# soedinglab/spacedust

Measured on AMD Instinct MI355X. Metric: clustersearch throughput (genome-pairs/s; SW GCUPS alongside), higher is better.
Workload: dtype int16

## Files before the change

### include/spacedust_gpu.h

```cpp
#ifndef SPACEDUST_GPU_H
#define SPACEDUST_GPU_H

#include <stddef.h>
#include <stdint.h>

#ifdef __cplusplus
extern "C" {
#endif

enum {
    SD_OK = 0,
    SD_ENODEVICE = -1,
    SD_EHIP = -2,
    SD_EINVAL = -3,
    SD_ENOMEM = -4,
    SD_EUNSUPPORTED = -5,
    SD_EMISMATCH = -6
};

typedef struct sd_ctx sd_ctx;
typedef struct sd_seqset sd_seqset;
typedef struct sd_target sd_target;

int sd_ctx_create(int device, sd_ctx **out);
// ... 59 lines not shown
                                    uint32_t nPairs, const uint32_t *pairQ, const uint32_t *pairT, const uint16_t *pairDiag,
                                    const uint8_t *isIdentity, float seqIdThr, int32_t alnLenThr, uint32_t *outIdx, sd_sw_result *out,
                                    uint32_t *nOut, char *btPool, uint64_t btCap, uint64_t *btUsed);

int sd_sw_align_alt_batch(sd_ctx *ctx, const sd_sw_params *par, const sd_seqset *queries, const sd_seqset *targets, uint32_t nSeeds,
                          const uint32_t *seedQ, const uint32_t *seedT, const int32_t *tStart, const int32_t *tEnd,
                          const uint8_t *isIdentity, uint32_t maxAlt, float seqIdThr, int32_t alnLenThr, int32_t seqIdMode,
                          sd_sw_result *out, uint32_t *outCount, char *btPool, uint64_t btCap, uint64_t *btUsed);
int sd_sw_alt_last_stats(sd_ctx *ctx, uint64_t *groups, uint64_t *seedRounds, uint64_t *bytesCopied);

int sd_sw_set_cigar_pool(sd_ctx *ctx, int on);
int sd_sw_download_bytes(sd_ctx *ctx, uint64_t *recordBytes, uint64_t *poolBytes);

int sd_sw_set_narrow_final(sd_ctx *ctx, int on);
int sd_sw_set_shared_start(sd_ctx *ctx, int on);

int sd_selftest_sort_pairs(sd_ctx *ctx, const uint32_t *keys, const uint32_t *vals, uint32_t n, int beginBit, int endBit, uint32_t *outKeys,
                           uint32_t *outVals);
int sd_selftest_scan(sd_ctx *ctx, const uint32_t *in, uint32_t n, uint64_t *exclusiveSum, uint32_t *runningMax);
int sd_selftest_score_class(int kernel , int32_t n, int32_t tL, int shared, int32_t wideRowLimit,
                            uint32_t *klass, char *scope, size_t cap);
int sd_selftest_r2p_weights(sd_ctx *ctx, uint32_t nTasks, const uint32_t *nRows, const uint32_t *L, const uint8_t *cells, float *freq,
                            float *eff);

int sd_sw_align_batch_hostpath(sd_ctx *ctx, const sd_sw_params *par, const sd_seqset *queries, const sd_seqset *targets,
                               uint32_t nPairs, const uint32_t *pairQ, const uint32_t *pairT, const uint8_t *isIdentity,
                               sd_sw_result *out, char *btPool, uint64_t btCap, uint64_t *btUsed);

int sd_sw_score_batch(sd_ctx *ctx, const sd_sw_params *par, const sd_seqset *queries, const sd_seqset *targets,
                      uint32_t nPairs, const uint32_t *pairQ, const uint32_t *pairT, int lanes, int reverse,
                      const int32_t *qEnd, const int32_t *tEnd, int32_t *out);

int sd_sw_last_cells(sd_ctx *ctx, uint64_t *forwardCells, uint64_t *reverseCells, uint64_t *tracebackCells);

typedef struct {
    int32_t kmerSize;
// ... 419 lines not shown
```

### spacedust_amd/_lib.py

```python
import ctypes as C
import os

import numpy as np

HERE = os.path.dirname(os.path.abspath(__file__))
LIB_PATH = os.path.join(HERE, 'libsdgpu.so')

_vp = C.c_void_p


SD_OK, SD_ENODEVICE, SD_EHIP, SD_EINVAL, SD_ENOMEM, SD_EUNSUPPORTED, SD_EMISMATCH = 0, -1, -2, -3, -4, -5, -6


class SdError(RuntimeError):
    pass


class SwParams(C.Structure):
    _fields_ = [('gapOpen', C.c_int32), ('gapExtend', C.c_int32), ('matrix', C.c_int8 * 441), ('covMode', C.c_int32),
                ('covThr', C.c_float), ('evalThr', C.c_double), ('swMode', C.c_int32), ('dbResidues', C.c_uint64)]


class SwResult(C.Structure):
    _fields_ = [('score', C.c_int32), ('qStart', C.c_int32), ('qEnd', C.c_int32), ('tStart', C.c_int32),
# ... 223 lines not shown
        'sd_search_result_arrays': (C.c_int, [_vp] + [_vp] * 12),
        'sd_search_result_write_tsv': (C.c_int, [_vp, C.c_char_p, C.c_char_p, _vp, C.c_char_p, _vp, C.c_char_p, _vp, C.c_char_p, _vp,
                                                 C.c_int, C.c_int, C.c_uint64, C.POINTER(C.c_uint64), C.POINTER(C.c_uint64)]),
        'sd_search_result_records': (C.c_int, [_vp, _vp, C.c_uint64, C.POINTER(C.c_uint64)]),
        'sd_agg_records': (C.c_int, [_vp] * 7 + [_vp, C.c_uint64, C.POINTER(C.c_uint64)]),
        'sd_records_check': (C.c_int, [_vp, C.c_uint64, C.c_uint32, C.c_uint32, C.c_uint32, C.c_uint32, C.POINTER(C.c_uint64), C.POINTER(C.c_uint64)]),
        'sd_records_write_tsv': (C.c_int, [_vp, C.c_uint64, C.c_char_p, C.c_int, C.c_uint64, C.c_char_p, _vp, C.c_char_p, _vp, C.c_char_p, _vp,
                                           C.c_char_p, _vp, C.c_int, C.POINTER(C.c_uint64), C.POINTER(C.c_uint64)]),
        'sd_search_result_destroy': (None, [_vp]),
        'sd_search_stats': (C.c_int, [_vp, _vp, _vp]),
        'sd_search_download_bytes': (C.c_int, [_vp, C.POINTER(C.c_uint64), C.POINTER(C.c_uint64)]),
        'sd_sw_set_cigar_pool': (C.c_int, [_vp, C.c_int]),
        'sd_sw_download_bytes': (C.c_int, [_vp, C.POINTER(C.c_uint64), C.POINTER(C.c_uint64)]),
        'sd_sw_set_narrow_final': (C.c_int, [_vp, C.c_int]),
        'sd_sw_set_shared_start': (C.c_int, [_vp, C.c_int]),
        'sd_r2p_create': (C.c_int, [C.POINTER(_vp)]),
        'sd_r2p_destroy': (None, [_vp]),
        'sd_r2p_batch': (C.c_int, [_vp, C.POINTER(R2pParams), C.c_uint32] + [_vp] * 12),
        'sd_r2p_batch_device': (C.c_int, [_vp, _vp, C.POINTER(R2pParams), C.c_uint32] + [_vp] * 12),
        'sd_selftest_r2p_weights': (C.c_int, [_vp, C.c_uint32, _vp, _vp, _vp, _vp, _vp]),
        'sd_selftest_score_class': (C.c_int, [C.c_int, C.c_int32, C.c_int32, C.c_int, C.c_int32, C.POINTER(C.c_uint32), C.c_char_p, C.c_size_t]),
        'sd_shard_query_sets': (C.c_int, [_vp, C.c_uint32, C.c_uint32, C.c_uint32, _vp, C.POINTER(C.c_uint32)]),
        'sd_comm_unique_id': (C.c_int, [C.c_char_p]),
        'sd_comm_init': (C.c_int, [C.c_int, C.c_int, C.c_int, C.c_char_p, C.POINTER(_vp)]),
        'sd_comm_destroy': (None, [_vp]),
        'sd_comm_host_buffer': (C.c_int, [_vp, C.c_int, C.c_uint64, C.POINTER(_vp)]),
        'sd_comm_last_error': (C.c_char_p, [_vp]),
        'sd_search_set_records_sink': (C.c_int, [_vp, _vp, _vp]),
        'sd_gather_stream_begin': (C.c_int, [_vp, C.c_int, C.c_uint32, _vp, C.c_uint32, _vp, C.c_uint64, C.c_int, C.POINTER(_vp)]),
        'sd_gather_stream_end': (C.c_int, [_vp, _vp, _vp, C.POINTER(C.c_uint64)]),
# ... 61 lines not shown
```

### spacedust_amd/api.py

```python
import ctypes as C

import numpy as np

from . import _lib
from .cpus import effective_cpus
from ._lib import SdError, ptr


def _check(ctx, rc, what):
    if rc != 0:
        msg = ''
        if ctx is not None:
            msg = _lib.load().sd_last_error(ctx).decode(errors='replace')
        raise SdError('%s failed (%d): %s' % (what, rc, msg))


class Host:

    def __init__(self, threads=0):
        import os
        self.L = _lib.load()
        self.threads = threads or effective_cpus()
        h = C.c_void_p()
        _check(None, self.L.sd_host_create(self.threads, C.byref(h)), 'sd_host_create')
# ... 81 lines not shown
        return out

    def evalue(self, db_residues, score, qlen):
        return self.L.sd_host_evalue(db_residues, float(score), float(qlen))

    def bitscore(self, score):
        return self.L.sd_host_bitscore(float(score))

    def score_class(self, kernel, n, tl, shared, wide_row_limit):
        klass = C.c_uint32()
        if not hasattr(self, '_scope_buf'):
            self._scope_buf = C.create_string_buffer(48)
        _check(None, self.L.sd_selftest_score_class(kernel, n, tl, int(shared), wide_row_limit, C.byref(klass), self._scope_buf, 48),
               'sd_selftest_score_class')
        return klass.value, self._scope_buf.value.decode()


def uncompress_cigar(c):
    out, n = [], 0
    for ch in c:
        if '0' <= ch <= '9':
            n = n * 10 + ord(ch) - 48
        else:
            out.append(ch * (n if n else 1))
            n = 0
    return ''.join(out)


def swapresults(entries, first_db_residues, second_db_keys, eval_thr=0.001, gap_open=11, gap_extend=1, want_counts=False):
    L = _lib.load()
# ... 333 lines not shown
        out = np.zeros(len(hq), _lib.RESCORE_DTYPE)
        _check(self.h, self.L.sd_rescore_diagonal_batch(self.h, C.byref(par), queries.h, targets.h, len(hq), ptr(hq), ptr(ht), ptr(hd),
                                                        ptr(out)), 'sd_rescore_diagonal_batch')
        return out

    def set_cigar_pool(self, on=True):
        _check(self.h, self.L.sd_sw_set_cigar_pool(self.h, 1 if on else 0), 'sd_sw_set_cigar_pool')
        self._cigar_pool = bool(on)

    def set_narrow_final(self, on=True):
        _check(self.h, self.L.sd_sw_set_narrow_final(self.h, 1 if on else 0), 'sd_sw_set_narrow_final')

    def set_shared_start(self, on=True):
        _check(self.h, self.L.sd_sw_set_shared_start(self.h, 1 if on else 0), 'sd_sw_set_shared_start')

    def sw_download_bytes(self):
        a, b = C.c_uint64(), C.c_uint64()
        self.L.sd_sw_download_bytes(self.h, C.byref(a), C.byref(b))
        return a.value, b.value

    def sw_cells(self):
        f, r, t = C.c_uint64(), C.c_uint64(), C.c_uint64()
        self.L.sd_sw_last_cells(self.h, C.byref(f), C.byref(r), C.byref(t))
        return f.value, r.value, t.value

    def __del__(self):
        try:
            h, self.h = self.h, None
            if h:
                self.L.sd_ctx_destroy(h)
# ... 483 lines not shown
```

### spacedust_amd/csrc/cli/sd_mod_iter.cpp

```cpp
#include "sd_align_core.h"
#include "sd_cli.h"
#include "sd_pref_core.h"

#include <algorithm>
#include <atomic>
#include <chrono>
#include <climits>
#include <cmath>
#include <condition_variable>
#include <cstdio>
#include <cstdlib>
#include <cstring>
#include <memory>
#include <mutex>
#include <omp.h>
#include <string>
#include <sys/resource.h>
#include <thread>
#include <vector>

namespace sdcli {

namespace {

// ... 43 lines not shown

struct Worker {
    sd_ctx *ctx = nullptr;
    sd_host *host = nullptr;
    sd_r2p *r2p = nullptr;
    int threads = 1;
    QueryChunk Q;
    std::vector<uint8_t> failed;
    AlignChunk C;
    std::vector<uint32_t> mark;
    uint32_t stamp = 0;
    ~Worker() {
        if (r2p) sd_r2p_destroy(r2p);
        if (ctx) sd_sw_set_narrow_final(ctx, 0);
        if (ctx) sd_sw_set_shared_start(ctx, 0);
        if (ctx) sd_ctx_destroy(ctx);
        if (host) sd_host_destroy(host);
    }
};

double quantE(double v) {
    char text[32];
    double back = v;
    sd_host_quantise_3e(v, text, &back);
    return back;
}

int failChunk(ChunkOut &o, int rc, const std::string &what, sd_ctx *ctx) {
    o.rc = rc;
    o.err = what + " failed (" + std::to_string(rc) + ")";
// ... 255 lines not shown
    nWorkers = std::max(1, std::min(nWorkers, 8));
    uint32_t chunkQ = (uint32_t) std::max<long long>(1, a.integer("--iter-chunk-queries", getenv("SD_ITER_CHUNK") ? atoi(getenv("SD_ITER_CHUNK")) : 1500));
    const int perWorker = std::max(1, std::min(threads, (threads * 3 / 2 + nWorkers - 1) / nWorkers));
    std::vector<std::unique_ptr<Worker> > workers;
    for (int w = 0; w < nWorkers; w++) {
        workers.emplace_back(new Worker());
        Worker &W = *workers.back();
        W.threads = perWorker;
        int rc = sd_ctx_create(device, &W.ctx);
        if (rc != SD_OK) return failNoDevice(rc);
        if (sd_host_create(perWorker, &W.host) != SD_OK) return fail("sd_host_create failed");
        if (sd_r2p_create(&W.r2p) != SD_OK) return fail("sd_r2p_create failed");
        if (S.profile) sd_profile_enable(W.ctx, 1);
        sd_sw_set_narrow_final(W.ctx, (getenv("SD_SW_NARROW_FINAL") && atoi(getenv("SD_SW_NARROW_FINAL")) == 0) ? 0 : 1);
        sd_sw_set_shared_start(W.ctx, (getenv("SD_SW_SHARED_START") && atoi(getenv("SD_SW_SHARED_START")) == 0) ? 0 : 1);
    }
    uint64_t indexEntries = 0;
    TargetH seqTarget, profTarget;
    SeqSetH tset;
    {
        sd_ctx *c0 = workers[0]->ctx;
        uint64_t st[2] = {0, 0};
        if (int rc = buildTarget(host.h, c0, S.pfSeq, tdb->residues.data(), tdb->offsets.data(), tdb->n, &seqTarget.t, st)) return rc;
        indexEntries = st[0];
        info(a, "Index table k-mer threshold: %d at k-mer size %d\nIndex statistics\nEntries:          %llu\n", S.pfSeq.kmerThr, S.pfSeq.k,
             (unsigned long long) st[0]);
        if (numIt > 1) {
            if (int rc = buildTarget(host.h, c0, S.pfProf, tdb->residues.data(), tdb->offsets.data(), tdb->n, &profTarget.t, st, std::string(),
                                     "sd_target_build (profile searches)"))
                return rc;
// ... 420 lines not shown
```

### spacedust_amd/csrc/hip/sd_common.h

```cpp
#ifndef SD_COMMON_H
#define SD_COMMON_H

#include <hip/hip_runtime.h>

#include <cstdarg>
#include <cstdint>
#include <cstdio>
#include <cstring>
#include <algorithm>
#include <ctime>
#include <sys/prctl.h>
#include <map>
#include <mutex>
#include <string>
#include <vector>

#include "spacedust_gpu.h"

struct sd_profile_entry {
    double ms = 0.0;
    uint64_t launches = 0;
};

struct sd_ctx {
    int device = 0;
    hipStream_t stream = nullptr;
    std::string lastError;
    bool profiling = false;
    std::map<std::string, sd_profile_entry> profile;
    hipEvent_t evStart = nullptr, evStop = nullptr;
    bool biasTablesUploaded = false;
    hipEvent_t evSync = nullptr;
    uint64_t cellsFwd = 0, cellsRev = 0, cellsTb = 0;
    uint64_t cellsUngapped = 0;
    uint64_t altGroups = 0, altSeedRounds = 0, altBytes = 0;
    const sd_sw_result *alignDevRes = nullptr;
    size_t alignDevResN = 0;
    bool cigarPool = false;
    bool sharedStart = false;
    bool narrowFinal = false;
    uint64_t d2hRecordBytes = 0, d2hPoolBytes = 0;
    struct ExpandState {
        uint64_t nPairs = 0, runsRead = 0, bytesWritten = 0;
        uint32_t nAB = 0;
        const int32_t *abStartA = nullptr, *abStartB = nullptr, *bcStartB = nullptr, *bcStartC = nullptr;
        const uint64_t *abRunOff = nullptr, *bcRowOff = nullptr, *bcRunOff = nullptr, *pairOff = nullptr;
        const uint32_t *abRuns = nullptr, *bcRuns = nullptr, *abCluster = nullptr;
        const sd_expand_result *res = nullptr;
    } expand;
    hipDeviceProp_t prop;
    struct WsEntry { void *p = nullptr; size_t bytes = 0; };
    std::map<std::string, WsEntry> ws;
    std::map<std::string, WsEntry> pinned;
    struct ProfPending { std::string name; hipEvent_t a = nullptr, b = nullptr; };
// ... 343 lines not shown
```

### spacedust_amd/csrc/hip/sd_sw.hip

```cpp
#include "sd_common.h"
#include <unistd.h>


#include <algorithm>
#include <cmath>
#include <cstring>
#include <memory>
#include <omp.h>
#include <numeric>

#include "../host/sd_host.h"
#include "sd_sw_pk.h"

namespace {

using sdpk::SwTask;
using sdpk::NARROW_EXACT;

template <int RT>
__global__ void __launch_bounds__(64)
sw_score_kernel(const SwTask *__restrict__ tasks, uint32_t nTasks, const uint8_t *__restrict__ qRes,
                const int8_t *__restrict__ qBias, const uint8_t *__restrict__ tRes, const int8_t *__restrict__ mat,
                int go, int ge, int32_t *__restrict__ out, uint2 *__restrict__ boundary,
                const uint32_t *__restrict__ order ,
// ... 451 lines not shown
        }
        going = going && !bad && (i > 0 || j > 0);
    }
    if (!have || l != 0) return;
    if (bad || i != 0 || j != 0) {
        res[2 * id] = -1;
        return;
    }
    ids += (q[0] == t[0]);
    *--o = 'M';
    len++;
    res[2 * id] = len;
    res[2 * id + 1] = ids;
}

template <bool PROF>
__global__ void __launch_bounds__(64)
sw_traceback_narrow_kernel(TbTask *__restrict__ tasks, uint32_t nTasks, const uint8_t *__restrict__ qRes,
                           const int8_t *__restrict__ qBias, const uint8_t *__restrict__ tRes, const int8_t *__restrict__ mat,
                           int go, int ge, int qCap, int tCap, char *__restrict__ bt, int32_t *__restrict__ res,
                           const uint32_t *__restrict__ order, const int8_t *__restrict__ qProf ) {
    extern __shared__ uint8_t ldsRaw[];
    __shared__ int8_t smat[441];
    for (int i = threadIdx.x; i < 441; i += 64) smat[i] = mat[i];
    const int grp = threadIdx.x >> 5, l = threadIdx.x & 31;
    const uint32_t lid = blockIdx.x * 2 + grp;
    const bool have = lid < nTasks;
    const uint32_t id = have ? (order ? order[lid] : lid) : 0;
    TbTask tk;
    if (have) tk = tasks[id];
    else { tk.qLen = 0; tk.tLen = 0; tk.band = 1; tk.score = 0; tk.maxv = 0; tk.qAbs = 0; tk.tAbs = 0; tk.slot = 0; tk.dirOff = 0; tk.btOff = 0; }
    const int qLen = tk.qLen, tLen = tk.tLen;
    const size_t perTask = (size_t) 16 * qCap + 2 * (size_t) qCap + tCap;
    uint8_t *dirs = ldsRaw + grp * perTask;
    uint8_t *sq = dirs + (size_t) 16 * qCap;
    int8_t *scb = (int8_t *) (sq + qCap);
    uint8_t *st = (uint8_t *) (scb + qCap);
    for (int x = l; x < qLen; x += 32) {
        sq[x] = qRes[tk.qAbs + x];
        scb[x] = qBias[tk.qAbs + x];
    }
    for (int x = l; x < tLen; x += 32) st[x] = tRes[tk.tAbs + x];
    __syncthreads();

    const int NEG = -(1 << 28);
    int band = tk.band, maxv = tk.maxv;
    bool reached = false;
    for (;;) {
        const int width = band * 2 + 3;
        const bool fits = width <= 32;
        int hb = 0, eb = 0;
        const int rows = (fits && !reached) ? qLen : 0;
        const int rowsOther = __shfl_xor(rows, 32, 64);
        const int nRows = max(rows, rowsOther);
        auto cellOps = [&](int row, int &qv, int &tv, int &cbv) {
            int r = row < qLen ? row : qLen - 1;
            r = r > 0 ? r : 0;
            const int x0 = (r - band) > 0 ? (r - band) : 0;
            int jn = x0 + l - 1;
            jn = jn >= tLen ? tLen - 1 : jn;
            jn = jn > 0 ? jn : 0;
            tv = st[jn];
            qv = 0;
            cbv = 0;
            if (!PROF) {
                qv = sq[r];
                cbv = scb[r];
            }
        };
        auto cellLook = [&](int row, int qv, int tv) -> int {
            int r = row < qLen ? row : qLen - 1;
            r = r > 0 ? r : 0;
            if (PROF) return (int) qProf[(tk.qAbs + (uint64_t) r) * 21 + (tv < 21 ? tv : 20)];
            return (int) smat[21 * qv + tv];
        };
        int qb, tb, cbb;
        cellOps(0, qb, tb, cbb);
        int sNext = cellLook(0, qb, tb), cNext = cbb;
        cellOps(1, qb, tb, cbb);
        for (int i = 0; i < nRows; i++) {
            const bool live = i < rows;
            const int sCur = sNext, cCur = cNext;
            sNext = cellLook(i + 1, qb, tb);
            cNext = cbb;
            cellOps(i + 2, qb, tb, cbb);
            const int xi = (i - band) > 0 ? (i - band) : 0;
            const int delta = (i - band) >= 1 ? 1 : 0;
            int end = tLen - 1;
            end = end < i + band ? end : i + band;
            const int edge = end + 1 < width - 1 ? end + 1 : width - 1;
            const int W = end - xi + 1;
            const bool zeroed = live && (l == 0 || l == edge);
            hb = zeroed ? 0 : hb;
            eb = zeroed ? 0 : eb;
            const int hbUp = dppZ(hb, 0x130), ebUp = dppZ(eb, 0x130), hbDn = dppZ(hb, 0x138);
            const int hE = delta ? hbUp : hb, eE = delta ? ebUp : eb, hD = delta ? hb : hbDn;
            const int u = l;
            const bool valid = live && u >= 1 && u <= W;
            const int t1 = i == 0 ? -go : hE - go;
            const int t2 = i == 0 ? -ge : eE - ge;
            const int eNew = t1 > t2 ? t1 : t2;
            const bool dirE = t1 > t2;
            const int e1 = eNew > 0 ? eNew : 0;
            const int diag = hD + sCur + cCur;
            const int T = e1 > diag ? e1 : diag;
            int incl = valid ? T + ge * u + 1 : 0, o;
            o = dppZ(incl, 0x111); incl = incl > o ? incl : o;
            o = dppZ(incl, 0x112); incl = incl > o ? incl : o;
            o = dppZ(incl, 0x114); incl = incl > o ? incl : o;
            o = dppZ(incl, 0x118); incl = incl > o ? incl : o;
            o = dppI(0, incl, 0x142, 0xa); incl = incl > o ? incl : o;
            int excl = dppZ(incl, 0x138);
            excl = l == 0 ? 0 : excl;
            const int gx = excl - go - 1;
            const int g = (-ge) > gx ? (-ge) : gx;
            const int f = g - ge * (u - 1);
            const int hcv = T > f ? T : f;
            int hcP = dppZ(hcv, 0x138), fP = dppZ(f, 0x138);
            hcP = u <= 1 ? 0 : hcP;
            fP = u <= 1 ? 0 : fP;
            const bool dirF = (hcP - go) > (fP - ge);
            const int f1 = f > 0 ? f : 0;
            const int tmp1 = e1 > f1 ? e1 : f1;
            int code = (dirE ? 1 : 0) | (dirF ? 2 : 0) | ((tmp1 > diag) ? ((e1 > f1) ? 4 : 8) : 0);
            code = valid ? code : 0;
            eb = valid ? eNew : eb;
            hb = valid ? hcv : hb;
            maxv = (valid && hcv > maxv) ? hcv : maxv;
            const int codeUp = dppZ(code, 0x130);
            if (valid && (u & 1)) dirs[(size_t) 16 * i + ((u - 1) >> 1)] = (uint8_t) (code | (codeUp << 4));
        }
        if (!reached && fits) {
#pragma unroll
            for (int off = 16; off >= 1; off >>= 1) {
                const int o2 = __shfl_xor(maxv, off, 32);
                maxv = o2 > maxv ? o2 : maxv;
            }
            if (maxv >= tk.score) reached = true;
            else band *= 2;
        }
        const bool done = reached || band * 2 + 3 > 32 || !have;
        const bool doneOther = __shfl_xor(done ? 1 : 0, 32, 64) != 0;
        if (done && doneOther) break;
    }
    __syncthreads();
    if (have && l == 0) {
        tasks[id].maxv = maxv;
        tasks[id].band = band;
        if (!reached) res[2 * id] = -2;
    }
    const int width_d = band * 2 + 1;
    int i = qLen - 1, j = tLen - 1, state = 2;
    char *o = bt + tk.btOff + (qLen + tLen + 2);
    int len = 0, ids = 0;
    bool bad = false;
    bool going = have && reached && (i > 0 || j > 0);
    const int sh = grp * 32;
    while (__ballot(going)) {
        {
            const int ii = i - l, jj = j - l;
            bool ok = going && state == 2 && (ii > 0 || jj > 0) && ii >= 0 && jj >= 0;
            int x = ii - band;
            x = x > 0 ? x : 0;
            x = jj - x;
            ok = ok && x >= 0 && x < width_d;
            bool same = false;
            if (ok) {
                const int byte = dirs[(size_t) 16 * ii + (x >> 1)];
                const int code = (x & 1) ? (byte >> 4) : (byte & 15);
                ok = (code & 12) == 0;
                same = sq[ii] == st[jj];
            }
            const uint32_t okMask = (uint32_t) (__ballot(ok) >> sh);
            const uint32_t sameMask = (uint32_t) (__ballot(same) >> sh);
            const int run = okMask == 0xFFFFFFFFu ? 32 : __builtin_ctz(~okMask);
            const uint32_t runMask = run == 32 ? 0xFFFFFFFFu : ((1u << run) - 1u);
            if (l < run) o[-1 - l] = 'M';
            ids += __builtin_popcount(sameMask & runMask);
            i -= run;
            j -= run;
            o -= run;
            len += run;
        }
        if (going && (i > 0 || j > 0)) {
            if (i < 0 || j < 0) bad = true;
            int x = i - band;
            x = x > 0 ? x : 0;
            x = j - x;
            if (x < 0 || x >= width_d) bad = true;
            if (!bad) {
                const int byte = dirs[(size_t) 16 * i + (x >> 1)];
                const int code = (x & 1) ? (byte >> 4) : (byte & 15);
                int dcode;
                const int dE = (code & 1) ? 3 : 2, dF = (code & 2) ? 5 : 4;
                if (state == 0) dcode = dE;
                else if (state == 1) dcode = dF;
                else dcode = (code & 4) ? dE : ((code & 8) ? dF : 1);
                char c;
                switch (dcode) {
                    case 1: ids += (sq[i] == st[j]); --i; --j; state = 2; c = 'M'; break;
                    case 2: --i; state = 0; c = 'I'; break;
                    case 3: --i; state = 2; c = 'I'; break;
                    case 4: --j; state = 1; c = 'D'; break;
                    default: --j; state = 2; c = 'D'; break;
                }
                --o;
// ... 481 lines not shown
        while (qLen > TB_CLASSES[ci].cap) ci++;
        const int tries = band <= 1 ? 4 : (band <= 3 ? 3 : (band <= 7 ? 2 : 1));
        return ci * 4096u + (uint32_t) (4 - tries) * 1024u + (uint32_t) (1023 - min(max(qLen - 1, 0), 1023));
    }
    const unsigned long long work = (unsigned long long) ((2 * band + 1 + 31) / 32) * (unsigned long long) qLen;
    return tbBandClass(band) * 4096u + (uint32_t) (4095 - (int) min(work >> 3, 4095ull));
}
__device__ __forceinline__ uint64_t tbDirBytes(int band, int qLen, int tLen) {
    if (tbNarrow(band, qLen, tLen)) return 0ull;
    const uint32_t ci = tbBandClass(band);
    if (ci == TB_GLOBAL)
        return (tbGlobalIntBytes(band) + (uint64_t) (band * 2 + 1) * (uint64_t) qLen + 31) & ~15ull;
    return ((uint64_t) (TB_CLASSES[ci].cap - 3) * (uint64_t) qLen + 31) & ~15ull;
}
void launchTbNarrow(sd_ctx *ctx, const sd_seqset *q, const sd_seqset *t, const int8_t *dMat, int go, int ge, const TbClass &cls, TbTask *dTb,
                    uint32_t cnt, char *dBt, int32_t *dTbRes, const uint32_t *order) {
    const int qCap = cls.cap, tCap = qCap + 16;
    const size_t ldsBytes = 2 * ((size_t) 16 * qCap + 2 * (size_t) qCap + tCap);
    auto *kernel = q->dProf ? sw_traceback_narrow_kernel<true> : sw_traceback_narrow_kernel<false>;
    hipLaunchKernelGGL(kernel, dim3((cnt + 1) / 2), dim3(64), ldsBytes, ctx->stream, dTb, cnt, q->dRes, q->dBias, t->dRes, dMat, go, ge, qCap,
                       tCap, dBt, dTbRes, order, (const int8_t *) q->dProf);
}
void launchTbBand(sd_ctx *ctx, const sd_seqset *q, const sd_seqset *t, const int8_t *dMat, int go, int ge, const TbClass &cls,
                  int maxWidthLoop, TbTask *dTb, uint32_t cnt, int8_t *dDir, char *dBt, int32_t *dTbRes, const uint32_t *order) {
    const bool global = cls.cap == 0;
    const int ldsStride = global ? INT_MAX : cls.cap + 1;
    const size_t ldsBytes = global ? 0 : (size_t) 2 * 3 * ldsStride * sizeof(int32_t);
    auto *band = global ? (q->dProf ? sw_traceback_kernel<true, true> : sw_traceback_kernel<false, true>)
                        : (q->dProf ? sw_traceback_kernel<true, false> : sw_traceback_kernel<false, false>);
    hipLaunchKernelGGL(band, dim3((cnt + 1) / 2), dim3(64), ldsBytes, ctx->stream, dTb, cnt, q->dRes, q->dBias, t->dRes, dMat, go, ge, ldsStride,
                       dDir, dBt, dTbRes, order, maxWidthLoop, (const int8_t *) q->dProf);
    auto *walk = global ? sw_traceback_walk_kernel<true> : sw_traceback_walk_kernel<false>;
    hipLaunchKernelGGL(walk, dim3((cnt + 256 / TBW_LANES - 1) / (256 / TBW_LANES)), dim3(256), 0, ctx->stream, dTb, cnt, q->dRes, t->dRes, dDir,
                       dBt, dTbRes, order);
}

// ... 879 lines not shown
    SD_HIP(ctx, wsGet(ctx, "al.tbres", N * 2, &w.dTbRes));
    SD_HIP(ctx, wsGet(ctx, "al.err", 4, &w.dErr));
    SD_HIP(ctx, wsGet(ctx, "al.tasks", N, &w.dTasks));
    SD_HIP(ctx, wsGet(ctx, "al.tb", N, &w.dTb));
    SD_HIP(ctx, wsGet(ctx, "al.res", N, &w.dRes));
    ctx->alignDevRes = w.dRes;
    ctx->alignDevResN = N;
    SD_HIP(ctx, wsGet(ctx, "al.scana", N + 1, &w.dScanA));
    SD_HIP(ctx, wsGet(ctx, "al.scanb", N + 1, &w.dScanB));
    SD_HIP(ctx, wsGet(ctx, "al.dirbytes", N + 1, &w.dDirBytes));
    SD_HIP(ctx, wsGet(ctx, "al.diroff", N + 1, &w.dDirOff));
    SD_HIP(ctx, wsGet(ctx, "al.btbytes", N + 1, &w.dBtBytes));
    SD_HIP(ctx, wsGet(ctx, "al.btoff", N + 1, &w.dBtOff));
    SD_HIP(ctx, wsGet(ctx, "al.btlen", N + 1, &w.dBtLen));
    SD_HIP(ctx, wsGet(ctx, "al.dense", N + 1, &w.dDense));
    SD_HIP(ctx, wsGet(ctx, "al.cells", 4, &w.dCells));
    SD_HIP(ctx, hipMemcpyAsync(w.dMat, a.par->matrix, 441, hipMemcpyHostToDevice, ctx->stream));
    SD_HIP(ctx, hipMemcpyAsync(w.dPQ, a.pairQ, N * sizeof(uint32_t), hipMemcpyHostToDevice, ctx->stream));
    SD_HIP(ctx, hipMemcpyAsync(w.dPT, a.pairT, N * sizeof(uint32_t), hipMemcpyHostToDevice, ctx->stream));
    if (a.isIdentity) SD_HIP(ctx, hipMemcpyAsync(w.dIdent, a.isIdentity, N, hipMemcpyHostToDevice, ctx->stream));
    else SD_HIP(ctx, hipMemsetAsync(w.dIdent, 0, N, ctx->stream));
    SD_HIP(ctx, hipMemcpyAsync(w.dMinBias, queries->dProf ? queries->hProfBias.data() : queries->hMinBias.data(),
                               queries->n * sizeof(int32_t), hipMemcpyHostToDevice, ctx->stream));
    SD_HIP(ctx, hipMemsetAsync(w.dErr, 0, 4 * sizeof(int), ctx->stream));
    SD_HIP(ctx, hipMemsetAsync(w.dCells, 0, 4 * sizeof(unsigned long long), ctx->stream));
    SD_HIP(ctx, hipMemsetAsync(w.dOut32, 0, N * 3 * sizeof(int32_t), ctx->stream));
    SD_HIP(ctx, hipMemsetAsync(w.dOut16, 0, N * 3 * sizeof(int32_t), ctx->stream));
    SD_HIP(ctx, hipMemsetAsync(w.dOutRev, 0, N * 3 * sizeof(int32_t), ctx->stream));
    SD_HIP(ctx, hipMemsetAsync(w.dBtLen, 0, (N + 1) * sizeof(uint64_t), ctx->stream));
    return SD_OK;
}

static int runTracebackRounds(sd_ctx *ctx, const AlignCall &a, const AlignWs &w) {
    const sd_seqset *queries = a.queries, *targets = a.targets;
    const uint32_t nPairs = a.nPairs;
    const size_t N = w.N;
    const int go = a.par->gapOpen, ge = a.par->gapExtend;
    uint64_t SCRATCH_BUDGET = 16ull << 30;
    {
        size_t freeB = 0, totalB = 0;
// ... 34 lines not shown
        }
        int8_t *dDir = nullptr;
        if (wsGet(ctx, "tb.dir", std::min<uint64_t>(dirTotal, SCRATCH_BUDGET) + 64, &dDir) != hipSuccess) {
            (void) hipGetLastError();
            if (SCRATCH_BUDGET <= (256ull << 20) || budgetRaised)
                return sdFail(ctx, SD_ENOMEM, "traceback direction scratch: out of device memory (%llu bytes for one round)",
                              (unsigned long long) std::min<uint64_t>(dirTotal, SCRATCH_BUDGET));
            SCRATCH_BUDGET /= 2;
            continue;
        }
        for (uint32_t ci = 0; ci < N_TB_CLASSES; ci++) {
            const uint32_t begin = hb[ci], cnt = hb[ci + 1] - hb[ci];
            if (cnt == 0) continue;
            const TbClass &cls = TB_CLASSES[ci];
            ProfScope ps(ctx, cls.scope);
            if (ci < N_TB_NARROW) launchTbNarrow(ctx, queries, targets, w.dMat, go, ge, cls, w.dTb, cnt, w.dBt, w.dTbRes, w.dOrder + begin);
            else launchTbBand(ctx, queries, targets, w.dMat, go, ge, cls, std::max(0, cls.cap - 1), w.dTb, cnt, dDir, w.dBt, w.dTbRes, w.dOrder + begin);
        }
        SD_HIP(ctx, hipGetLastError());
        hipLaunchKernelGGL(k_tb_collect, dim3(w.grid), dim3(256), 0, ctx->stream, nPairs, w.dKeys, w.dVals, w.dTb, w.dTbRes, w.dDirBytes, w.dBtLen,
                           w.dRes, w.dErr, 4 * 65536, dKeysRound);
    }
    return sdFail(ctx, SD_EHIP, "traceback: tasks still pending after 4096 rounds");
}

static int printTracebackStats(sd_ctx *ctx, const AlignWs &w, uint32_t nPairs) {
    std::vector<TbTask> hT(nPairs);
    std::vector<uint64_t> hL(nPairs);
    SD_HIP(ctx, hipMemcpy(hT.data(), w.dTb, (size_t) nPairs * sizeof(TbTask), hipMemcpyDeviceToHost));
    SD_HIP(ctx, hipMemcpy(hL.data(), w.dBtLen, (size_t) nPairs * sizeof(uint64_t), hipMemcpyDeviceToHost));
    uint64_t nDone = 0, init6 = 0, init6final6 = 0, init6final14 = 0, final14 = 0;
// ... 53 lines not shown
static int downloadRecords(sd_ctx *ctx, const AlignCall &a, const AlignWs &w, bool narrowFinal, AlignRecords &rec) {
    const uint32_t nPairs = a.nPairs;
    const size_t N = w.N;
    const bool cigarPool = rec.cigarPool = ctx->cigarPool && a.btPool != nullptr;
    uint64_t *dCigLen = nullptr;
    if (cigarPool) {
        SD_HIP(ctx, wsGet(ctx, "al.ciglen", N + 1, &dCigLen));
        SD_HIP(ctx, hipMemsetAsync(dCigLen + nPairs, 0, (N + 1 - nPairs) * sizeof(uint64_t), ctx->stream));
        hipLaunchKernelGGL(k_bt_cigar<false>, dim3((nPairs + 3) / 4), dim3(256), 0, ctx->stream, nPairs, (const uint64_t *) w.dBtLen,
                           (const uint64_t *) nullptr, (const TbTask *) w.dTb, (const char *) w.dBt, (char *) nullptr, dCigLen, (sd_sw_result *) nullptr);
    }
    const int rc = devExclusiveScan(ctx, cigarPool ? dCigLen : w.dBtLen, w.dDense, N + 1);
    if (rc != SD_OK) return rc;
    uint64_t &poolBytes = rec.poolBytes = 0;
    int hErr[4] = {0, 0, 0, 0};
    unsigned long long hCells[4] = {0, 0, 0, 0};
    SD_HIP(ctx, sdD2H(ctx, &poolBytes, w.dDense + N, sizeof(uint64_t)));
    SD_HIP(ctx, sdD2H(ctx, hErr, w.dErr, sizeof(hErr)));
    SD_HIP(ctx, sdD2H(ctx, hCells, w.dCells, sizeof(hCells)));
    SD_HIP(ctx, sdStreamSync(ctx));
    if (hErr[0] == 1) return sdFail(ctx, SD_EMISMATCH, "Score of forward/backward SW differ (fatal in the reference, StripedSmithWaterman.cpp:466-473)");
    if (hErr[0] == 2) return sdFail(ctx, SD_EHIP, "Trace back error");
    ctx->cellsFwd = hCells[0];
    ctx->cellsRev = hCells[1];
    if (narrowFinal && ctx->profiling) {
        const double add[3] = {(double) hCells[2], (double) hCells[3], (double) (hCells[2] - hCells[3])};
        static const char *const names[3] = {"stat.sw_word_pairs", "stat.sw_word_wide", "stat.sw_word_narrow_final"};
        for (int x = 0; x < 3; x++) {
            sd_profile_entry &pe = ctx->profile[names[x]];
            pe.ms += add[x];
            pe.launches += 1;
        }
    }
    uint64_t identBytes = 0;
    if (a.isIdentity && a.btPool)
        for (uint32_t i = 0; i < nPairs; i++)
            if (a.isIdentity[i]) identBytes += cigarPool ? 8 : a.targets->hOff[a.pairT[i] + 1] - a.targets->hOff[a.pairT[i]];
    if (poolBytes > 0 && a.btPool == nullptr) return sdFail(ctx, SD_EINVAL, "swMode 2 needs a backtrace pool");
    if (poolBytes + identBytes > a.btCap && a.btPool) return sdFail(ctx, SD_ENOMEM, "backtrace pool too small");
    char *dPool = nullptr;
    SD_HIP(ctx, wsGet(ctx, "al.pool", poolBytes + 64, &dPool));
    if (poolBytes > 0 && cigarPool)
        hipLaunchKernelGGL(k_bt_cigar<true>, dim3((nPairs + 3) / 4), dim3(256), 0, ctx->stream, nPairs, (const uint64_t *) w.dBtLen,
                           (const uint64_t *) w.dDense, (const TbTask *) w.dTb, (const char *) w.dBt, dPool, (uint64_t *) nullptr, w.dRes);
    else if (poolBytes > 0)
// ... 207 lines not shown
    return SD_OK;
}

int sd_sw_set_narrow_final(sd_ctx *ctx, int on) {
    if (!ctx) return SD_EINVAL;
    ctx->narrowFinal = on != 0;
    return SD_OK;
}

int sd_sw_set_shared_start(sd_ctx *ctx, int on) {
    if (!ctx) return SD_EINVAL;
    ctx->sharedStart = on != 0;
    return SD_OK;
}

int sd_sw_download_bytes(sd_ctx *ctx, uint64_t *recordBytes, uint64_t *poolBytes) {
    if (!ctx) return SD_EINVAL;
    if (recordBytes) *recordBytes = ctx->d2hRecordBytes;
    if (poolBytes) *poolBytes = ctx->d2hPoolBytes;
    return SD_OK;
}

int sd_sw_align_batch(sd_ctx *ctx, const sd_sw_params *par, const sd_seqset *queries, const sd_seqset *targets,
                      uint32_t nPairs, const uint32_t *pairQ, const uint32_t *pairT, const uint8_t *isIdentity,
                      sd_sw_result *out, char *btPool, uint64_t btCap, uint64_t *btUsed) {
    return alignBatchImpl(ctx, {par, queries, targets, nPairs, pairQ, pairT, isIdentity, out, btPool, btCap, btUsed, nullptr, nullptr, nullptr, nullptr});
}

int sd_sw_align_batch_compact(sd_ctx *ctx, const sd_sw_params *par, const sd_seqset *queries, const sd_seqset *targets,
                              uint32_t nPairs, const uint32_t *pairQ, const uint32_t *pairT, const uint8_t *isIdentity,
// ... 49 lines not shown
        rc = devInclusiveMax(ctx, dIn.p, dMax.p, n);
        if (rc != SD_OK) return rc;
    }
    SD_HIP(ctx, hipStreamSynchronize(ctx->stream));
    SD_HIP(ctx, hipMemcpy(exclusiveSum, dOut.p, ((size_t) n + 1) * 8, hipMemcpyDeviceToHost));
    if (runningMax) SD_HIP(ctx, hipMemcpy(runningMax, dMax.p, (size_t) n * 4, hipMemcpyDeviceToHost));
    return SD_OK;
}

int sd_selftest_score_class(int kernel, int32_t n, int32_t tL, int shared, int32_t wideRowLimit, uint32_t *klass, char *scope, size_t cap) {
    if (kernel < SCORE_PK || kernel > SCORE_PK_START || n < 1 || tL < 1 || !klass || (cap && !scope)) return SD_EINVAL;
    const uint32_t ci = scoreClassOf(n, tL, kernel, wideRowLimit);
    const ScoreSide &side = shared && (ci < FIRST_INT32_CLASS || ci >= FIRST_START_CLASS) ? SCORE_CLASSES[ci].shared : SCORE_CLASSES[ci].unshared;
    *klass = ci;
    if (cap) snprintf(scope, cap, "%s", side.scope);
    return SD_OK;
}

int sd_sw_align_batch_best_by_group(sd_ctx *ctx, const sd_sw_params *par, const sd_seqset *queries, const sd_seqset *targets,
                                    uint32_t nPairs, const uint32_t *pairQ, const uint32_t *pairT, const uint16_t *pairDiag,
                                    const uint8_t *isIdentity, float seqIdThr, int32_t alnLenThr, uint32_t *outIdx, sd_sw_result *out,
                                    uint32_t *nOut, char *btPool, uint64_t btCap, uint64_t *btUsed) {
    if (!outIdx || !nOut || !targets) return SD_EINVAL;
    if (!targets->dGroupOf) return sdFail(ctx, SD_EINVAL, "sd_sw_align_batch_best_by_group: the target set has no groups (sd_seqset_set_groups)");
    const float bb[2] = {seqIdThr, (float) alnLenThr};
    return alignBatchImpl(ctx, {par, queries, targets, nPairs, pairQ, pairT, isIdentity, out, btPool, btCap, btUsed, outIdx, nOut, pairDiag, bb});
}

int sd_sw_align_batch_hostpath(sd_ctx *ctx, const sd_sw_params *par, const sd_seqset *queries, const sd_seqset *targets,
                      uint32_t nPairs, const uint32_t *pairQ, const uint32_t *pairT, const uint8_t *isIdentity,
// ... 226 lines not shown
```

### spacedust_amd/csrc/host/sd_search.cpp

```cpp
#include "sd_host.h"
#include "sd_target_build.h"
#include "spacedust_gpu.h"

#include <algorithm>
#include <chrono>
#include <condition_variable>
#include <cstdio>
#include <cstdlib>
#include <cstring>
#include <deque>
#include <fstream>
#include <functional>
#include <future>
#include <memory>
#include <mutex>
#include <string>
#include <thread>
#include <pthread.h>
#include <vector>

namespace {

double nowSec() {
    return std::chrono::duration<double>(std::chrono::steady_clock::now().time_since_epoch()).count();
// ... 459 lines not shown
            for (sd_ctx *c : al)
                if (c) sd_sw_set_narrow_final(c, 0);
        }
    } narrowFinalMode(s, !(getenv("SD_SW_NARROW_FINAL") && atoi(getenv("SD_SW_NARROW_FINAL")) == 0));
    struct SharedStartMode {
        sd_ctx *al[4];
        explicit SharedStartMode(sd_search *s_, bool on) : al{s_->ctxAl, s_->ctxAl2, s_->ctxAlMore[0], s_->ctxAlMore[1]} {
            for (sd_ctx *c : al)
                if (c) sd_sw_set_shared_start(c, on ? 1 : 0);
        }
        ~SharedStartMode() {
            for (sd_ctx *c : al)
                if (c) sd_sw_set_shared_start(c, 0);
        }
    } sharedStartMode(s, !(getenv("SD_SW_SHARED_START") && atoi(getenv("SD_SW_SHARED_START")) == 0));
    std::vector<uint32_t> qSetSize(Q->nSets, 0);
    if (aggregate)
        for (uint32_t i = 0; i < Q->n; i++)
            if (Q->setId[i] < Q->nSets) qSetSize[Q->setId[i]]++;
    if (aggregate) {
        uint32_t m = 0;
        for (uint32_t v : qSetSize) m = std::max(m, v);
        for (uint32_t v : s->tSetSize) m = std::max(m, v);
        for (uint32_t i = 0; i < Q->n; i++) m = std::max(m, Q->posInSet[i]);
        for (uint32_t i = 0; i < T.n; i++) m = std::max(m, T.posInSet[i]);
        if (s->lgamma.size() < (size_t) m + 8) {
            s->lgamma.resize((size_t) m + 8);
            sd_host_lgamma_table(s->lgamma.data(), (uint32_t) s->lgamma.size());
        }
    }
// ... 586 lines not shown
```

Baseline: 3062.

## Pack multiple band widths into one narrow traceback pass via rung ladder

New measurement: 3069 (median of 6 runs). Within noise of the previous version (+0.2%).

```diff
diff --git a/include/spacedust_gpu.h b/include/spacedust_gpu.h
--- a/include/spacedust_gpu.h
+++ b/include/spacedust_gpu.h
@@ -97,12 +97,14 @@
 
 int sd_sw_set_narrow_final(sd_ctx *ctx, int on);
 int sd_sw_set_shared_start(sd_ctx *ctx, int on);
+int sd_sw_set_tb_ladder(sd_ctx *ctx, int on);
 
 int sd_selftest_sort_pairs(sd_ctx *ctx, const uint32_t *keys, const uint32_t *vals, uint32_t n, int beginBit, int endBit, uint32_t *outKeys,
                            uint32_t *outVals);
 int sd_selftest_scan(sd_ctx *ctx, const uint32_t *in, uint32_t n, uint64_t *exclusiveSum, uint32_t *runningMax);
 int sd_selftest_score_class(int kernel , int32_t n, int32_t tL, int shared, int32_t wideRowLimit,
                             uint32_t *klass, char *scope, size_t cap);
+int sd_selftest_tb_rungs(int32_t band, int ladder, int32_t *n, int32_t *bands , int32_t *bases , int32_t *nextBand);
 int sd_selftest_r2p_weights(sd_ctx *ctx, uint32_t nTasks, const uint32_t *nRows, const uint32_t *L, const uint8_t *cells, float *freq,
                             float *eff);
 
diff --git a/spacedust_amd/_lib.py b/spacedust_amd/_lib.py
--- a/spacedust_amd/_lib.py
+++ b/spacedust_amd/_lib.py
@@ -261,6 +261,8 @@
         'sd_sw_download_bytes': (C.c_int, [_vp, C.POINTER(C.c_uint64), C.POINTER(C.c_uint64)]),
         'sd_sw_set_narrow_final': (C.c_int, [_vp, C.c_int]),
         'sd_sw_set_shared_start': (C.c_int, [_vp, C.c_int]),
+        'sd_sw_set_tb_ladder': (C.c_int, [_vp, C.c_int]),
+        'sd_selftest_tb_rungs': (C.c_int, [C.c_int32, C.c_int, C.POINTER(C.c_int32), C.POINTER(C.c_int32), C.POINTER(C.c_int32), C.POINTER(C.c_int32)]),
         'sd_r2p_create': (C.c_int, [C.POINTER(_vp)]),
         'sd_r2p_destroy': (None, [_vp]),
         'sd_r2p_batch': (C.c_int, [_vp, C.POINTER(R2pParams), C.c_uint32] + [_vp] * 12),
diff --git a/spacedust_amd/api.py b/spacedust_amd/api.py
--- a/spacedust_amd/api.py
+++ b/spacedust_amd/api.py
@@ -119,6 +119,12 @@
         _check(None, self.L.sd_selftest_score_class(kernel, n, tl, int(shared), wide_row_limit, C.byref(klass), self._scope_buf, 48),
                'sd_selftest_score_class')
         return klass.value, self._scope_buf.value.decode()
+
+    def tb_rungs(self, band, ladder=True):
+        n, nxt = C.c_int32(), C.c_int32()
+        bands, bases = (C.c_int32 * 3)(), (C.c_int32 * 3)()
+        _check(None, self.L.sd_selftest_tb_rungs(band, int(ladder), C.byref(n), bands, bases, C.byref(nxt)), 'sd_selftest_tb_rungs')
+        return tuple(bands[:n.value]), tuple(bases[:n.value]), nxt.value
 
 
 def uncompress_cigar(c):
@@ -482,6 +488,9 @@
     def set_shared_start(self, on=True):
         _check(self.h, self.L.sd_sw_set_shared_start(self.h, 1 if on else 0), 'sd_sw_set_shared_start')
 
+    def set_tb_ladder(self, on=True):
+        _check(self.h, self.L.sd_sw_set_tb_ladder(self.h, 1 if on else 0), 'sd_sw_set_tb_ladder')
+
     def sw_download_bytes(self):
         a, b = C.c_uint64(), C.c_uint64()
         self.L.sd_sw_download_bytes(self.h, C.byref(a), C.byref(b))
diff --git a/spacedust_amd/csrc/cli/sd_mod_iter.cpp b/spacedust_amd/csrc/cli/sd_mod_iter.cpp
--- a/spacedust_amd/csrc/cli/sd_mod_iter.cpp
+++ b/spacedust_amd/csrc/cli/sd_mod_iter.cpp
@@ -81,6 +81,7 @@
         if (r2p) sd_r2p_destroy(r2p);
         if (ctx) sd_sw_set_narrow_final(ctx, 0);
         if (ctx) sd_sw_set_shared_start(ctx, 0);
+        if (ctx) sd_sw_set_tb_ladder(ctx, 0);
         if (ctx) sd_ctx_destroy(ctx);
         if (host) sd_host_destroy(host);
     }
@@ -366,6 +367,7 @@
         if (S.profile) sd_profile_enable(W.ctx, 1);
         sd_sw_set_narrow_final(W.ctx, (getenv("SD_SW_NARROW_FINAL") && atoi(getenv("SD_SW_NARROW_FINAL")) == 0) ? 0 : 1);
         sd_sw_set_shared_start(W.ctx, (getenv("SD_SW_SHARED_START") && atoi(getenv("SD_SW_SHARED_START")) == 0) ? 0 : 1);
+        sd_sw_set_tb_ladder(W.ctx, (getenv("SD_TB_LADDER") && atoi(getenv("SD_TB_LADDER")) == 0) ? 0 : 1);
     }
     uint64_t indexEntries = 0;
     TargetH seqTarget, profTarget;
diff --git a/spacedust_amd/csrc/hip/sd_common.h b/spacedust_amd/csrc/hip/sd_common.h
--- a/spacedust_amd/csrc/hip/sd_common.h
+++ b/spacedust_amd/csrc/hip/sd_common.h
@@ -38,6 +38,7 @@
     size_t alignDevResN = 0;
     bool cigarPool = false;
     bool sharedStart = false;
+    bool tbLadder = false;
     bool narrowFinal = false;
     uint64_t d2hRecordBytes = 0, d2hPoolBytes = 0;
     struct ExpandState {
diff --git a/spacedust_amd/csrc/hip/sd_sw.hip b/spacedust_amd/csrc/hip/sd_sw.hip
--- a/spacedust_amd/csrc/hip/sd_sw.hip
+++ b/spacedust_amd/csrc/hip/sd_sw.hip
@@ -489,12 +489,27 @@
     res[2 * id + 1] = ids;
 }
 
+constexpr int TB_MAX_RUNGS = 3;
+__host__ __device__ __forceinline__ int tbRungCount(int band, bool ladder) {
+    int n = 1;
+    if (ladder && band <= 14)
+        for (int sum = 2 * band + 3, b = 2 * band; n < TB_MAX_RUNGS && sum + 2 * b + 3 <= 32; b *= 2) {
+            sum += 2 * b + 3;
+            n++;
+        }
+    return n;
+}
+__host__ __device__ __forceinline__ int tbRungBand(int band, int k) { return band << k; }
+__host__ __device__ __forceinline__ int tbRungBase(int band, int k) { return 2 * band * ((1 << k) - 1) + 4 * k; }
+constexpr int TB_RUNG_SEP = 1 << 24;
+
 template <bool PROF>
 __global__ void __launch_bounds__(64)
 sw_traceback_narrow_kernel(TbTask *__restrict__ tasks, uint32_t nTasks, const uint8_t *__restrict__ qRes,
                            const int8_t *__restrict__ qBias, const uint8_t *__restrict__ tRes, const int8_t *__restrict__ mat,
                            int go, int ge, int qCap, int tCap, char *__restrict__ bt, int32_t *__restrict__ res,
-                           const uint32_t *__restrict__ order, const int8_t *__restrict__ qProf ) {
+                           const uint32_t *__restrict__ order, const int8_t *__restrict__ qProf ,
+                           int ladder, unsigned long long *__restrict__ stat ) {
     extern __shared__ uint8_t ldsRaw[];
     __shared__ int8_t smat[441];
     for (int i = threadIdx.x; i < 441; i += 64) smat[i] = mat[i];
@@ -519,20 +534,28 @@
     __syncthreads();
 
     const int NEG = -(1 << 28);
-    int band = tk.band, maxv = tk.maxv;
+    int band = tk.band, maxv = tk.maxv, base = 0, passes = 0;
     bool reached = false;
+    const int gNone = (-ge) > (-go - 1) ? (-ge) : (-go - 1);
     for (;;) {
-        const int width = band * 2 + 3;
-        const bool fits = width <= 32;
-        int hb = 0, eb = 0;
+        const bool fits = band * 2 + 3 <= 32;
+        const int nRungs = tbRungCount(band, ladder != 0);
+        int rung = 0;
+#pragma unroll
+        for (int k = 1; k < TB_MAX_RUNGS; k++)
+            if (k < nRungs && l >= tbRungBase(band, k)) rung = k;
+        const int bandL = tbRungBand(band, rung), u = l - tbRungBase(band, rung), width = bandL * 2 + 3;
+        const int inclAdd = ge * u + 1 + rung * TB_RUNG_SEP, exclSub = rung * TB_RUNG_SEP + go + 1, fSub = ge * (u - 1);
+        int hb = 0, eb = 0, mx = 0;
         const int rows = (fits && !reached) ? qLen : 0;
+        passes += rows > 0 ? 1 : 0;
         const int rowsOther = __shfl_xor(rows, 32, 64);
         const int nRows = max(rows, rowsOther);
         auto cellOps = [&](int row, int &qv, int &tv, int &cbv) {
             int r = row < qLen ? row : qLen - 1;
             r = r > 0 ? r : 0;
-            const int x0 = (r - band) > 0 ? (r - band) : 0;
-            int jn = x0 + l - 1;
+            const int x0 = (r - bandL) > 0 ? (r - bandL) : 0;
+            int jn = x0 + u - 1;
             jn = jn >= tLen ? tLen - 1 : jn;
             jn = jn > 0 ? jn : 0;
             tv = st[jn];
@@ -559,18 +582,17 @@
             sNext = cellLook(i + 1, qb, tb);
             cNext = cbb;
             cellOps(i + 2, qb, tb, cbb);
-            const int xi = (i - band) > 0 ? (i - band) : 0;
-            const int delta = (i - band) >= 1 ? 1 : 0;
+            const int xi = (i - bandL) > 0 ? (i - bandL) : 0;
+            const int delta = (i - bandL) >= 1 ? 1 : 0;
             int end = tLen - 1;
-            end = end < i + band ? end : i + band;
+            end = end < i + bandL ? end : i + bandL;
             const int edge = end + 1 < width - 1 ? end + 1 : width - 1;
             const int W = end - xi + 1;
-            const bool zeroed = live && (l == 0 || l == edge);
+            const bool zeroed = live && (u == 0 || u == edge);
             hb = zeroed ? 0 : hb;
             eb = zeroed ? 0 : eb;
             const int hbUp = dppZ(hb, 0x130), ebUp = dppZ(eb, 0x130), hbDn = dppZ(hb, 0x138);
             const int hE = delta ? hbUp : hb, eE = delta ? ebUp : eb, hD = delta ? hb : hbDn;
-            const int u = l;
             const bool valid = live && u >= 1 && u <= W;
             const int t1 = i == 0 ? -go : hE - go;
             const int t2 = i == 0 ? -ge : eE - ge;
@@ -579,7 +601,7 @@
             const int e1 = eNew > 0 ? eNew : 0;
             const int diag = hD + sCur + cCur;
             const int T = e1 > diag ? e1 : diag;
-            int incl = valid ? T + ge * u + 1 : 0, o;
+            int incl = valid ? T + inclAdd : 0, o;
             o = dppZ(incl, 0x111); incl = incl > o ? incl : o;
             o = dppZ(incl, 0x112); incl = incl > o ? incl : o;
             o = dppZ(incl, 0x114); incl = incl > o ? incl : o;
@@ -587,9 +609,9 @@
             o = dppI(0, incl, 0x142, 0xa); incl = incl > o ? incl : o;
             int excl = dppZ(incl, 0x138);
             excl = l == 0 ? 0 : excl;
-            const int gx = excl - go - 1;
-            const int g = (-ge) > gx ? (-ge) : gx;
-            const int f = g - ge * (u - 1);
+            const int gx = excl - exclSub;
+            const int g = gNone > gx ? gNone : gx;
+            const int f = g - fSub;
             const int hcv = T > f ? T : f;
             int hcP = dppZ(hcv, 0x138), fP = dppZ(f, 0x138);
             hcP = u <= 1 ? 0 : hcP;
@@ -601,18 +623,28 @@
             code = valid ? code : 0;
             eb = valid ? eNew : eb;
             hb = valid ? hcv : hb;
-            maxv = (valid && hcv > maxv) ? hcv : maxv;
+            mx = (valid && hcv > mx) ? hcv : mx;
             const int codeUp = dppZ(code, 0x130);
-            if (valid && (u & 1)) dirs[(size_t) 16 * i + ((u - 1) >> 1)] = (uint8_t) (code | (codeUp << 4));
+            if (valid && (u & 1)) dirs[(size_t) 16 * i + ((l - 1) >> 1)] = (uint8_t) (code | (codeUp << 4));
         }
         if (!reached && fits) {
+            const int first = band;
+            int last = band;
 #pragma unroll
-            for (int off = 16; off >= 1; off >>= 1) {
-                const int o2 = __shfl_xor(maxv, off, 32);
-                maxv = o2 > maxv ? o2 : maxv;
+            for (int k = 0; k < TB_MAX_RUNGS; k++) {
+                int mk = rung == k ? mx : 0;
+#pragma unroll
+                for (int off = 16; off >= 1; off >>= 1) {
+                    const int o2 = __shfl_xor(mk, off, 32);
+                    mk = o2 > mk ? o2 : mk;
+                }
+                if (k < nRungs && !reached) {
+                    maxv = mk > maxv ? mk : maxv;
+                    last = tbRungBand(first, k);
+                    if (maxv >= tk.score) { reached = true; band = last; base = tbRungBase(first, k); }
+                }
             }
-            if (maxv >= tk.score) reached = true;
-            else band *= 2;
+            if (!reached) band = last * 2;
         }
         const bool done = reached || band * 2 + 3 > 32 || !have;
         const bool doneOther = __shfl_xor(done ? 1 : 0, 32, 64) != 0;
@@ -623,6 +655,10 @@
         tasks[id].maxv = maxv;
         tasks[id].band = band;
         if (!reached) res[2 * id] = -2;
+        if (stat) {
+            atomicAdd(stat, 1ull);
+            atomicAdd(stat + 1, (unsigned long long) passes);
+        }
     }
     const int width_d = band * 2 + 1;
     int i = qLen - 1, j = tLen - 1, state = 2;
@@ -641,7 +677,7 @@
             ok = ok && x >= 0 && x < width_d;
             bool same = false;
             if (ok) {
-                const int byte = dirs[(size_t) 16 * ii + (x >> 1)];
+                const int byte = dirs[(size_t) 16 * ii + ((base + x) >> 1)];
                 const int code = (x & 1) ? (byte >> 4) : (byte & 15);
                 ok = (code & 12) == 0;
                 same = sq[ii] == st[jj];
@@ -664,7 +700,7 @@
             x = j - x;
             if (x < 0 || x >= width_d) bad = true;
             if (!bad) {
-                const int byte = dirs[(size_t) 16 * i + (x >> 1)];
+                const int byte = dirs[(size_t) 16 * i + ((base + x) >> 1)];
                 const int code = (x & 1) ? (byte >> 4) : (byte & 15);
                 int dcode;
                 const int dE = (code & 1) ? 3 : 2, dF = (code & 2) ? 5 : 4;
@@ -1176,12 +1212,12 @@
     return ((uint64_t) (TB_CLASSES[ci].cap - 3) * (uint64_t) qLen + 31) & ~15ull;
 }
 void launchTbNarrow(sd_ctx *ctx, const sd_seqset *q, const sd_seqset *t, const int8_t *dMat, int go, int ge, const TbClass &cls, TbTask *dTb,
-                    uint32_t cnt, char *dBt, int32_t *dTbRes, const uint32_t *order) {
+                    uint32_t cnt, char *dBt, int32_t *dTbRes, const uint32_t *order, unsigned long long *dStat ) {
     const int qCap = cls.cap, tCap = qCap + 16;
     const size_t ldsBytes = 2 * ((size_t) 16 * qCap + 2 * (size_t) qCap + tCap);
     auto *kernel = q->dProf ? sw_traceback_narrow_kernel<true> : sw_traceback_narrow_kernel<false>;
     hipLaunchKernelGGL(kernel, dim3((cnt + 1) / 2), dim3(64), ldsBytes, ctx->stream, dTb, cnt, q->dRes, q->dBias, t->dRes, dMat, go, ge, qCap,
-                       tCap, dBt, dTbRes, order, (const int8_t *) q->dProf);
+                       tCap, dBt, dTbRes, order, (const int8_t *) q->dProf, ctx->tbLadder ? 1 : 0, dStat);
 }
 void launchTbBand(sd_ctx *ctx, const sd_seqset *q, const sd_seqset *t, const int8_t *dMat, int go, int ge, const TbClass &cls,
                   int maxWidthLoop, TbTask *dTb, uint32_t cnt, int8_t *dDir, char *dBt, int32_t *dTbRes, const uint32_t *order) {
@@ -2091,7 +2127,7 @@
     SD_HIP(ctx, wsGet(ctx, "al.btoff", N + 1, &w.dBtOff));
     SD_HIP(ctx, wsGet(ctx, "al.btlen", N + 1, &w.dBtLen));
     SD_HIP(ctx, wsGet(ctx, "al.dense", N + 1, &w.dDense));
-    SD_HIP(ctx, wsGet(ctx, "al.cells", 4, &w.dCells));
+    SD_HIP(ctx, wsGet(ctx, "al.cells", 6, &w.dCells));
     SD_HIP(ctx, hipMemcpyAsync(w.dMat, a.par->matrix, 441, hipMemcpyHostToDevice, ctx->stream));
     SD_HIP(ctx, hipMemcpyAsync(w.dPQ, a.pairQ, N * sizeof(uint32_t), hipMemcpyHostToDevice, ctx->stream));
     SD_HIP(ctx, hipMemcpyAsync(w.dPT, a.pairT, N * sizeof(uint32_t), hipMemcpyHostToDevice, ctx->stream));
@@ -2100,7 +2136,7 @@
     SD_HIP(ctx, hipMemcpyAsync(w.dMinBias, queries->dProf ? queries->hProfBias.data() : queries->hMinBias.data(),
                                queries->n * sizeof(int32_t), hipMemcpyHostToDevice, ctx->stream));
     SD_HIP(ctx, hipMemsetAsync(w.dErr, 0, 4 * sizeof(int), ctx->stream));
-    SD_HIP(ctx, hipMemsetAsync(w.dCells, 0, 4 * sizeof(unsigned long long), ctx->stream));
+    SD_HIP(ctx, hipMemsetAsync(w.dCells, 0, 6 * sizeof(unsigned long long), ctx->stream));
     SD_HIP(ctx, hipMemsetAsync(w.dOut32, 0, N * 3 * sizeof(int32_t), ctx->stream));
     SD_HIP(ctx, hipMemsetAsync(w.dOut16, 0, N * 3 * sizeof(int32_t), ctx->stream));
     SD_HIP(ctx, hipMemsetAsync(w.dOutRev, 0, N * 3 * sizeof(int32_t), ctx->stream));
@@ -2165,7 +2201,8 @@
             if (cnt == 0) continue;
             const TbClass &cls = TB_CLASSES[ci];
             ProfScope ps(ctx, cls.scope);
-            if (ci < N_TB_NARROW) launchTbNarrow(ctx, queries, targets, w.dMat, go, ge, cls, w.dTb, cnt, w.dBt, w.dTbRes, w.dOrder + begin);
+            if (ci < N_TB_NARROW) launchTbNarrow(ctx, queries, targets, w.dMat, go, ge, cls, w.dTb, cnt, w.dBt, w.dTbRes, w.dOrder + begin,
+                                                  ctx->profiling ? w.dCells + 4 : nullptr);
             else launchTbBand(ctx, queries, targets, w.dMat, go, ge, cls, std::max(0, cls.cap - 1), w.dTb, cnt, dDir, w.dBt, w.dTbRes, w.dOrder + begin);
         }
         SD_HIP(ctx, hipGetLastError());
@@ -2249,7 +2286,7 @@
     if (rc != SD_OK) return rc;
     uint64_t &poolBytes = rec.poolBytes = 0;
     int hErr[4] = {0, 0, 0, 0};
-    unsigned long long hCells[4] = {0, 0, 0, 0};
+    unsigned long long hCells[6] = {0, 0, 0, 0, 0, 0};
     SD_HIP(ctx, sdD2H(ctx, &poolBytes, w.dDense + N, sizeof(uint64_t)));
     SD_HIP(ctx, sdD2H(ctx, hErr, w.dErr, sizeof(hErr)));
     SD_HIP(ctx, sdD2H(ctx, hCells, w.dCells, sizeof(hCells)));
@@ -2264,6 +2301,14 @@
         for (int x = 0; x < 3; x++) {
             sd_profile_entry &pe = ctx->profile[names[x]];
             pe.ms += add[x];
+            pe.launches += 1;
+        }
+    }
+    if (ctx->profiling) {
+        static const char *const names[2] = {"stat.tb_narrow_tasks", "stat.tb_narrow_passes"};
+        for (int x = 0; x < 2; x++) {
+            sd_profile_entry &pe = ctx->profile[names[x]];
+            pe.ms += (double) hCells[4 + x];
             pe.launches += 1;
         }
     }
@@ -2501,6 +2546,12 @@
     return SD_OK;
 }
 
+int sd_sw_set_tb_ladder(sd_ctx *ctx, int on) {
+    if (!ctx) return SD_EINVAL;
+    ctx->tbLadder = on != 0;
+    return SD_OK;
+}
+
 int sd_sw_download_bytes(sd_ctx *ctx, uint64_t *recordBytes, uint64_t *poolBytes) {
     if (!ctx) return SD_EINVAL;
     if (recordBytes) *recordBytes = ctx->d2hRecordBytes;
@@ -2580,6 +2631,18 @@
     const ScoreSide &side = shared && (ci < FIRST_INT32_CLASS || ci >= FIRST_START_CLASS) ? SCORE_CLASSES[ci].shared : SCORE_CLASSES[ci].unshared;
     *klass = ci;
     if (cap) snprintf(scope, cap, "%s", side.scope);
+    return SD_OK;
+}
+
+int sd_selftest_tb_rungs(int32_t band, int ladder, int32_t *n, int32_t *bands, int32_t *bases, int32_t *nextBand) {
+    if (band < 1 || band > (1 << 24) || !n || !bands || !bases || !nextBand) return SD_EINVAL;
+    const int nr = tbRungCount(band, ladder != 0);
+    *n = nr;
+    for (int k = 0; k < TB_MAX_RUNGS; k++) {
+        bands[k] = k < nr ? tbRungBand(band, k) : 0;
+        bases[k] = k < nr ? tbRungBase(band, k) : 0;
+    }
+    *nextBand = tbRungBand(band, nr - 1) * 2;
     return SD_OK;
 }
 
diff --git a/spacedust_amd/csrc/host/sd_search.cpp b/spacedust_amd/csrc/host/sd_search.cpp
--- a/spacedust_amd/csrc/host/sd_search.cpp
+++ b/spacedust_amd/csrc/host/sd_search.cpp
@@ -497,6 +497,17 @@
                 if (c) sd_sw_set_shared_start(c, 0);
         }
     } sharedStartMode(s, !(getenv("SD_SW_SHARED_START") && atoi(getenv("SD_SW_SHARED_START")) == 0));
+    struct TbLadderMode {
+        sd_ctx *al[4];
+        explicit TbLadderMode(sd_search *s_, bool on) : al{s_->ctxAl, s_->ctxAl2, s_->ctxAlMore[0], s_->ctxAlMore[1]} {
+            for (sd_ctx *c : al)
+                if (c) sd_sw_set_tb_ladder(c, on ? 1 : 0);
+        }
+        ~TbLadderMode() {
+            for (sd_ctx *c : al)
+                if (c) sd_sw_set_tb_ladder(c, 0);
+        }
+    } tbLadderMode(s, !(getenv("SD_TB_LADDER") && atoi(getenv("SD_TB_LADDER")) == 0));
     std::vector<uint32_t> qSetSize(Q->nSets, 0);
     if (aggregate)
         for (uint32_t i = 0; i < Q->n; i++)
```
